# TzuYaoHuang/WaterLily.jl

Hardware: AMD Instinct MI355X
Metric: cells*steps/sec (3D TGV) ; smoother HBM GB/s vs peak (higher is better)
Workload: dtype f32; 1 GPU; 3D Taylor-Green vortex 512^3 Float32, wall-bounded, Re=1600, NoBody, remeasure=false (BASELINE configs[4] domain on 1 GPU); size=512, resjac=630, resjac_redo=0

## Files before the change

### include/wlhip.h

```cpp
#ifndef WLHIP_H
#define WLHIP_H
#include <stddef.h>
#include <stdint.h>

#ifdef __cplusplus
extern "C" {
#endif

#define WL_EINVAL (-1)
#define WL_ENOGPU (-2)
#define WL_ELEVELS (-3)
#define WL_ECOMM (-4)

typedef struct wl_grid {
  int32_t D;
  int32_t nx, ny, nz;
  int32_t k0, k1;
  int32_t gk;
  int32_t gnz;
} wl_grid;

enum { WL_QUICK = 0, WL_VANLEER = 1, WL_CDS = 2 };

int wl_init(int device);
// ... 75 lines not shown
float* wl_mg_level_field(const wl_mg* mg, int level, const char* name);
int wl_mg_vcycle(wl_mg* mg, int level, float omega, void* stream);
int wl_mg_smooth(wl_mg* mg, int level, int it, float omega, void* stream);
int wl_mg_level_is_const(const wl_mg* mg, int level);
int wl_mg_smoother_kind(const wl_mg* mg, int level);
int wl_mg_set_fused(wl_mg* mg, int on);
int wl_mg_solve(wl_mg* mg, double tol, int itmx, int* host_n, double* host_r1, float* host_rinf, void* stream);
int wl_mg_history(const wl_mg* mg, int16_t* host_out, int cap);
int wl_mg_last_log(const wl_mg* mg, double* host_r1, double* host_rinf, double* host_omega, int cap);
int wl_mg_shift_path(const wl_mg* mg);

typedef struct wl_sim wl_sim;
typedef struct wl_sim_desc {
  int32_t D;
  int32_t dims[3];
  float uBC[3];
  float nu, dt0;
  uint32_t perdir_mask;
  int32_t exitBC;
  int32_t scheme;
  int32_t has_body;
  float *u, *u0, *f, *p, *sigma, *V, *mu0, *mu1;
  float *us;
} wl_sim_desc;
int wl_sim_create(wl_sim** out, const wl_sim_desc* desc);
int wl_sim_create_on(wl_sim** out, const wl_sim_desc* desc, wl_mg* mg);
int wl_sim_destroy(wl_sim* s);
float* wl_sim_field(wl_sim* s, const char* name);
wl_mg* wl_sim_pois(wl_sim* s);
int wl_sim_grid(const wl_sim* s, wl_grid* out);
int wl_sim_init_flow(wl_sim* s, void* stream);
int wl_sim_set_option(wl_sim* s, const char* name, int value);
int wl_reset_process_options(void);
int wl_sim_set_forcing(wl_sim* s, const float* U1, const float* a0, const float* a1);
int wl_accelerate(float* r, const wl_grid* g, const float a[3], void* stream);
int wl_sim_set_sgs(wl_sim* s, int model, float Cs, float Delta);
int wl_sim_update(wl_sim* s, void* stream);
int wl_sim_mom_step(wl_sim* s, void* stream);
int wl_sim_mom_steps(wl_sim* s, int n, void* stream);
int wl_sim_dt(const wl_sim* s, float* host_out, int cap);
double wl_sim_time(const wl_sim* s);
float wl_sim_dt_last(const wl_sim* s);
int wl_sim_set_dt_last(wl_sim* s, float dt);
int wl_sim_phase(wl_sim* s, int phase, void* stream);
int wl_sim_apply_ic(wl_sim* s, int kind, void* stream);
int wl_sim_measure_sphere(wl_sim* s, const float* host_center, float R, float eps, void* stream);
enum { WL_BODY_SPHERE = 1, WL_BODY_PLANE = 2 };
typedef struct wl_body { int32_t kind; float c[3]; float R; float m[3]; float V[3]; } wl_body;
int wl_measure_body(float* sigma, float* mu0, float* mu1, float* V, const wl_grid* g, const wl_body* host_body, float eps, int exitBC, uint32_t perdir_mask, void* stream);
int wl_pressure_force_body(const float* p, const wl_grid* g, const wl_body* host_body, double out[3], void* stream);
int wl_viscous_force_body(const float* u, const wl_grid* g, float nu, const wl_body* host_body, double out[3], void* stream);
int wl_pressure_moment_body(const float* host_x0, const float* p, const wl_grid* g, const wl_body* host_body, double out[3], void* stream);
int wl_viscous_moment_body(const float* host_x0, const float* u, const wl_grid* g, float nu, const wl_body* host_body, double out[3], void* stream);
int wl_sim_pressure_moment_body(wl_sim* s, const float* host_x0, const wl_body* host_body, double out[3], void* stream);
int wl_sim_viscous_moment_body(wl_sim* s, const float* host_x0, const wl_body* host_body, double out[3], void* stream);
int wl_sim_measure_body(wl_sim* s, const wl_body* host_body, float eps, void* stream);
int wl_sim_pressure_force_body(wl_sim* s, const wl_body* host_body, double out[3], void* stream);
int wl_sim_viscous_force_body(wl_sim* s, const wl_body* host_body, double out[3], void* stream);
int wl_sim_pressure_force_sphere(wl_sim* s, const float* host_center, float R, double* host_out, void* stream);
int wl_sim_viscous_force_sphere(wl_sim* s, const float* center, float R, double* out, void* stream);

int wl_sim_flow_stats(wl_sim* s, const float* host_U, double out[3], void* stream);
int wl_sim_flow_fields(wl_sim* s, const float* host_U, float* ke, float* omega3, float* omega_mag, float* lambda2, void* stream);

int wl_interp(float* out, const float* arr, const wl_grid* g, const float* x, size_t n, int ncomp, void* hip_stream);
int wl_sim_sample(wl_sim* s, const float* x, size_t n, float* u_out, float* p_out, void* hip_stream);
// ... 66 lines not shown
```

### waterlily.jl_amd/__init__.py

```python
from ._lib import LIB_PATH, SIGNATURES, WlError, lib
from .core import (BC_, CDS, QUICK, VANLEER, L2, exitBC_, inside, jl_zeros, loc, perBC_, to_device, to_host)
from .flow import BDIM_, CFL, Flow, conv_diff_, mom_correct_, mom_predict_, mom_project_, mom_step_, scale_u_, sgs, sgs_, udf_
from .poisson import (pcg_, poisson_solver_, GaussSeidelRB_, Jacobi_, L1, Linf, MultiLevelPoisson, Poisson, increment_, mult_, norms, prolongate_,
                      residual_, restrict_, restrictL_, set_diag_, smooth_, update_)
from .metrics import (MeanFlow, curl_, flow_fields_, flow_stats, helicity_, ke_, lambda2_, load_checkpoint, omega_, omega_mag_, omega_theta_,
                      save_checkpoint)
from .interp import advect_, interp, interp_
from .simulation import (FusedSimulation, Simulation, measure_, pressure_force, pressure_moment, viscous_force,
                         viscous_moment)
from . import bodies
from .bodies import Body, RigidMap, SdfLattice, SetBody, setmap
```

### waterlily.jl_amd/_lib.py

```python
import ctypes as C
import os

_HERE = os.path.dirname(os.path.abspath(__file__))
LIB_PATH = os.environ.get("WLHIP_LIB") or os.path.join(_HERE, "libwlhip.so")


class wl_grid(C.Structure):
    _fields_ = [("D", C.c_int32), ("nx", C.c_int32), ("ny", C.c_int32), ("nz", C.c_int32),
                ("k0", C.c_int32), ("k1", C.c_int32), ("gk", C.c_int32), ("gnz", C.c_int32)]


class wl_body(C.Structure):
    _fields_ = [("kind", C.c_int32), ("c", C.c_float * 3), ("R", C.c_float), ("m", C.c_float * 3), ("V", C.c_float * 3)]


def make_body(body, D):
    name = body[0]
    pad = lambda v: [float(x) for x in v] + [0.0] * (3 - len(v))
    b = wl_body()
    if name == "sphere":
        b.kind, b.R, m, rest = 1, float(body[2]), [1.0] * D, body[3:]
    elif name == "cylinder":
        b.kind, b.R, m, rest = 1, float(body[2]), [0.0 if k == int(body[3]) else 1.0 for k in range(D)], body[4:]
    elif name == "plane":
# ... 118 lines not shown
    "wl_sim_set_forcing": (i32, [P, C.POINTER(f32), C.POINTER(f32), C.POINTER(f32)]),
    "wl_accelerate": (i32, [P, G, C.POINTER(f32), P]),
    "wl_sim_set_sgs": (i32, [P, i32, f32, f32]),
    "wl_sim_mom_step": (i32, [P, P]),
    "wl_sim_mom_steps": (i32, [P, i32, P]),
    "wl_sim_dt": (i32, [P, C.POINTER(f32), i32]),
    "wl_sim_time": (f64, [P]),
    "wl_sim_dt_last": (f32, [P]),
    "wl_sim_set_dt_last": (i32, [P, f32]),
    "wl_sim_phase": (i32, [P, i32, P]),
    "wl_sim_apply_ic": (i32, [P, i32, P]),
    "wl_sim_measure_sphere": (i32, [P, C.POINTER(f32), f32, f32, P]),
    "wl_comm_rccl_unique_id": (i32, [C.c_char_p]),
    "wl_comm_rccl_create": (i32, [C.POINTER(P), i32, i32, C.c_char_p]),
    "wl_comm_callbacks_create": (i32, [C.POINTER(P), i32, i32, P, P, P]),
    "wl_comm_rccl_available": (i32, []),
    "wl_comm_rccl_add_async": (i32, [P, C.c_char_p]),
    "wl_comm_set_loopback": (i32, [P, i32]),
    "wl_comm_set_virtual": (i32, [P, i32, i32]),
    "wl_comm_set_virtual_transport": (i32, [P, i32]),
    "wl_comm_set_periodic": (i32, [P, i32]),
    "wl_comm_halo_async": (i32, [P, P, G, i32, i32, P]),
    "wl_comm_combine_test": (i32, [P, P, P, P]),
    "wl_comm_destroy": (i32, [P]),
    "wl_comm_rank": (i32, [P]),
    "wl_comm_size": (i32, [P]),
    "wl_comm_stats": (i32, [P, C.POINTER(C.c_int64)]),
    "wl_halo_exchange": (i32, [P, P, G, i32, i32, P]),
    "wl_allgather_planes": (i32, [P, P, G, i32, P]),
    "wl_grid_slab": (i32, [G, i32, C.POINTER(C.c_int32), i32, i32, i32]),
    "wl_sim_create_slab": (i32, [C.POINTER(P), C.POINTER(wl_sim_desc), P]),
    "wl_launch_count": (C.c_long, []),
    "wl_reset_process_options": (i32, []),
    "wl_placement_scores": (i32, [C.POINTER(C.c_double), i32]),
    "wl_sim_counter": (i32, [P, C.c_char_p, C.POINTER(C.c_long)]),
    "wl_prof_enable": (i32, [i32]),
    "wl_prof_read": (i32, [i32, C.POINTER(i32), C.POINTER(f64)]),
    "wl_sim_pressure_force_sphere": (i32, [P, C.POINTER(f32), f32, C.POINTER(f64), P]),
    "wl_measure_body": (i32, [P, P, P, P, G, C.POINTER(wl_body), f32, i32, C.c_uint32, P]),
    "wl_pressure_force_body": (i32, [P, G, C.POINTER(wl_body), C.POINTER(f64), P]),
    "wl_viscous_force_body": (i32, [P, G, f32, C.POINTER(wl_body), C.POINTER(f64), P]),
    "wl_pressure_moment_body": (i32, [C.POINTER(f32), P, G, C.POINTER(wl_body), C.POINTER(f64), P]),
    "wl_viscous_moment_body": (i32, [C.POINTER(f32), P, G, f32, C.POINTER(wl_body), C.POINTER(f64), P]),
    "wl_sim_pressure_moment_body": (i32, [P, C.POINTER(f32), C.POINTER(wl_body), C.POINTER(f64), P]),
    "wl_sim_viscous_moment_body": (i32, [P, C.POINTER(f32), C.POINTER(wl_body), C.POINTER(f64), P]),
    "wl_sim_measure_body": (i32, [P, C.POINTER(wl_body), f32, P]),
    "wl_sim_pressure_force_body": (i32, [P, C.POINTER(wl_body), C.POINTER(f64), P]),
    "wl_sim_viscous_force_body": (i32, [P, C.POINTER(wl_body), C.POINTER(f64), P]),
    "wl_bodyset_measure_points": (i32, [C.POINTER(wl_bodyset), i32, C.POINTER(f32), i32, f32, C.POINTER(f32), C.POINTER(f32), C.POINTER(f32), P]),
    "wl_measure_bodyset": (i32, [P, P, P, P, G, C.POINTER(wl_bodyset), f32, i32, C.c_uint32, P]),
    "wl_pressure_force_bodyset": (i32, [C.POINTER(f32), P, G, C.POINTER(wl_bodyset), C.POINTER(f64), P]),
    "wl_viscous_force_bodyset": (i32, [C.POINTER(f32), P, G, f32, C.POINTER(wl_bodyset), C.POINTER(f64), P]),
    "wl_sim_measure_bodyset": (i32, [P, C.POINTER(wl_bodyset), f32, P]),
    "wl_sim_pressure_force_bodyset": (i32, [P, C.POINTER(f32), C.POINTER(wl_bodyset), C.POINTER(f64), P]),
    "wl_sim_viscous_force_bodyset": (i32, [P, C.POINTER(f32), C.POINTER(wl_bodyset), C.POINTER(f64), P]),
    "wl_sim_viscous_force_sphere": (i32, [P, C.POINTER(f32), f32, C.POINTER(f64), P]),
    "wl_sdf_lattice_create": (i32, [C.POINTER(P), i32, C.POINTER(C.c_int32), C.POINTER(f32), P]),
    "wl_sdf_lattice_destroy": (i32, [P]),
    "wl_sdf_lattice_id": (i32, [P]),
    "wl_sim_set_force_record": (i32, [P, C.POINTER(wl_bodyset), C.POINTER(f32), i32]),
    "wl_sim_read_forces": (i32, [P, C.POINTER(f64), i32, C.POINTER(i32), C.POINTER(i32)]),
    "wl_sim_forces_bodyset": (i32, [P, C.POINTER(f32), C.POINTER(wl_bodyset), C.POINTER(f64), P]),
    "wl_interp": (i32, [P, P, G, P, sz, i32, P]),
    "wl_sim_sample": (i32, [P, P, sz, P, P, P]),
    "wl_sim_set_probes": (i32, [P, C.POINTER(f32), i32, i32]),
    "wl_sim_read_probes": (i32, [P, C.POINTER(f32), i32, C.POINTER(i32), C.POINTER(i32)]),
# ... 36 lines not shown
```

### waterlily.jl_amd/csrc/wl_common.hpp

```cpp
#pragma once
#include <functional>
#include <cstdlib>
#include <hip/hip_runtime.h>
#include <stdint.h>

#include <mutex>
#include <string>
#include <vector>

#include "../../include/wlhip.h"
#include "../../include/wlhip_bench.h"

#define WL_WAVE 64
#define WL_BLOCK 256

void wl_set_error(const std::string& s);
#define WL_HIP(call)                                                                      \
  do {                                                                                    \
    hipError_t e__ = (call);                                                              \
    if (e__ != hipSuccess) {                                                              \
      wl_set_error(std::string(#call) + ": " + hipGetErrorString(e__));                   \
      return (int)e__;                                                                    \
    }                                                                                     \
  } while (0)
// ... 214 lines not shown
                   float dt, float pre, float post, const ConstL& cl, hipStream_t s, int ka = -(1 << 30), int kb = 1 << 30, bool q1 = true, BcFold* fold = nullptr);
int conv_q1(float* Phi, const float* u, const GridX& g, float nu, unsigned per, int scheme, hipStream_t s);
bool conv_z_ok(const GridX& g, unsigned per);
int conv_diff_z(float* f, const float* u_adv, const float* u0, const float* mu0, float* u_out, const GridX& g, float nu, int scheme, float dt, float pre, float post, hipStream_t s);
int bdim(float* u, const float* u0, float* f, const float* V, const float* mu0, const float* mu1, const GridX& g, float dt, float pre, float post, hipStream_t s);
int accelerate(float* r, const GridX& g, const float* a, hipStream_t s);
int exit_bc_single(const GridX& G, float* u, const float* u0, double* sc, float dt, hipStream_t s);
int exit_bc_slab_sum(const GridX& G, const float* u, double* sum, int mode, hipStream_t s);
int exit_bc_slab_update(const GridX& G, float* u, const float* u0, const double* gsum, double* sc, float dt, int mode, hipStream_t s);
int copy_exit_face(float* dst, const float* src, const GridX& G, hipStream_t s);
int sgs(float* f, float* sigma, const float* u, const GridX& g, float Cs, float Delta, hipStream_t s);
int metrics_fields(const float* u, const GridX& g, const float* U, float* ke, float* w3, float* wmag, float* l2, hipStream_t s);
int metrics_omega_theta(float* out, const float* u, const GridX& g, const float* z, const float* c, hipStream_t s);
int metrics_curl(float* out, const float* u, const GridX& g, int i, hipStream_t s);
int metrics_helicity(float* out, const float* u, const float* w3, const GridX& g, hipStream_t s);
int metrics_stats_dev(const float* u, const GridX& g, const float* U, const RedWs& ws, hipStream_t s);
int interp_points(const float* vec, const float* sca, const GridX& g, const float* x, size_t n, float* out_v, long ldv, float* out_s, long lds, hipStream_t s);
int advect(float* x, float* x_prev, const float* u0, const float* u1, const GridX& g, size_t n, float dt, unsigned per, hipStream_t s);
int bc_vec_fn(float* a, const float* Ub, const GridX& g, int saveexit, unsigned per, hipStream_t s);
int add_field(float* r, const float* gfield, size_t n, hipStream_t s);
int meanflow_update(float* P, float* U, float* UU, const float* p, const float* u, const GridX& g, float e, hipStream_t s);
int meanflow_uu(float* tau, const float* UU, const float* U, const GridX& g, hipStream_t s);
int bc_zplanes(float* u, const GridX& g, float U2, hipStream_t s);
void conv_tile_enable(int on, int chunk);
void conv_tile_min(long tile_planes);
bool conv_tile_ok(const GridX& g, unsigned per, int nplanes);
int conv_tile(const float* u_adv, const GridX& g, float nu, int scheme, int ka, int kb, const void* bdim_args, hipStream_t s);
void conv_flux_enable(int on);
bool conv_flux_on();
bool conv_proj_ok(const GridX& g, unsigned per);
int conv_flux(const float* u_adv, const GridX& g, float nu, int scheme, int ka, int kb, int zchunk, const void* bdim_args, hipStream_t s);
void conv_march_enable(int on);
void jacobi_march_enable(int on);
bool conv_march_ok(const GridX& g);
int conv_march(float* r, const float* u, const GridX& g, float nu, unsigned per, int scheme, int kfirst, int klast, const void* bdim_args, hipStream_t s);
int bdim_f(float* f, const float* u0, const float* V, const GridX& g, float dt, hipStream_t s);
int bdim_u(float* u, const float* f, const float* V, const float* mu0, const float* mu1, const GridX& g, float pre, float post, hipStream_t s, const unsigned char* far = nullptr);
size_t body_mask_bytes(const GridX& g);
int conv_diff_bdim_body(float* f, const float* u_adv, float* Phi, const float* u0, const float* mu0, float* u_out, const GridX& g, float nu, unsigned per, int scheme,
                        float dt, float pre, float post, const unsigned char* near, const unsigned char* needf, const unsigned char* m0var, int nbm, int store_all, hipStream_t s,
                        int dz0 = 0, int dz1 = -1);
struct MaskCensus { long near = 0, needf_only = 0, m0var_only = 0, clean_in_box = 0; };
int body_masks_planes(const unsigned char* near, const unsigned char* needf, const unsigned char* m0var, const GridX& g, int* dz, hipStream_t s,
                      const int* box = nullptr, MaskCensus* census = nullptr);
void conv_body_tile_enable(int on);
long conv_body_tile_launches();
int body_masks_nbm(const GridX& g);
int body_masks(unsigned char* near, unsigned char* needf, unsigned char* m0var, const float* V, const float* mu1, const float* mu0, const GridX& g, hipStream_t s);
int bdim_near(float* uout, const float* uin, const float* u0, float* f, const float* V, const float* mu0, const float* mu1, const GridX& g, float dt, float pre, float post,
              const unsigned char* near, int nbm, const int* box, hipStream_t s);
int body_masks_box(const unsigned char* near, const GridX& g, int* box, hipStream_t s);
int body_mask(unsigned char* far, const float* V, const float* mu1, const GridX& g, hipStream_t s);
int scale_u(float* u, const GridX& g, float sc, hipStream_t s);
int div(float* z, const float* u, const GridX& g, hipStream_t s);
int div_scale(float* z, float* x, const float* u, const GridX& g, float dt, hipStream_t s);
int project(float* u, const float* L, const float* x, const GridX& g, hipStream_t s);
int cfl_dev(const float* u, float* sigma, const GridX& g, const RedWs& ws, int slot_f, hipStream_t s);

int set_diag(float* D, float* iD, const float* L, const GridX& g, hipStream_t s);
int mult(float* z, const float* L, const float* D, const float* x, const GridX& g, hipStream_t s);
int residual(float* r, const float* x, const float* z, const float* L, const float* D, const float* iD, const GridX& g, const RedWs& ws, hipStream_t s);
int residual_part(float* r, const float* x, const float* z, const float* L, const float* D, const float* iD, const GridX& g, const RedWs& ws, hipStream_t s);
int mean_shift(float* r, const GridX& g, const RedWs& ws, hipStream_t s);
int div_residual(float* z, float* xout, float* r, const float* x, const float* u, const float* L, const float* D, const float* iD, const GridX& g, float dt, const RedWs& ws, const ConstL& cl, hipStream_t s);
int div_residual_split(float* z, float* xout, float* r, const float* x, const float* u, const float* L, const float* D, const float* iD, const GridX& g, float dt, const RedWs& ws,
                       const ConstL& near, const ConstL& far, int na, int nb, hipStream_t s);
// ... 56 lines not shown
```

### waterlily.jl_amd/csrc/wl_poisson.hip

```cpp
#include <vector>

#include "wl_common.hpp"
#include "wl_bcfold.hpp"
#include "wl_pdefer.hpp"

namespace {

template <int D>
__device__ __forceinline__ float Ax(const GridX& g, long o, const float* __restrict__ L, const float* __restrict__ Dg, const float* __restrict__ x) {
  float s = x[o] * Dg[o];
  s += (x[o - 1] * L[o] + x[o + 1] * L[o + 1]);
  s += (x[o - g.sy] * L[g.cs + o] + x[o + g.sy] * L[g.cs + o + g.sy]);
  if (D == 3) s += (x[o - g.sz] * L[2 * g.cs + o] + x[o + g.sz] * L[2 * g.cs + o + g.sz]);
  return s;
}

template <int D>
__global__ void k_set_diag(GridX g, float* __restrict__ Dg, float* __restrict__ iD, const float* __restrict__ L) {
  int i, j; long m; int pz;
  wl_tile(g, m, pz);
  if (!cell_ij(g, m, i, j) || !interior_ij(g, i, j)) return;
  const long o = m + (long)(g.k0 + pz) * g.sz;
  float s = 0.f;
  s -= (L[o] + L[o + 1]);
// ... 581 lines not shown
  float s = r[o];
  s -= (E(o - 1) * L[o] + E(o + 1) * L[o + 1]);
  s -= (E(o - g.sy) * L[g.cs + o] + E(o + g.sy) * L[g.cs + o + g.sy]);
  if (D == 3) s -= (E(o - g.sz) * L[2 * g.cs + o] + E(o + g.sz) * L[2 * g.cs + o + g.sz]);
  eps[o] = s * iD[o];
}
template <int D>
__global__ void k_jacobi_pp_cl(GridX g, float* __restrict__ rout, const float* __restrict__ r, float* __restrict__ x, float w, wl::ConstL cl, int xzero) {
  __shared__ float sDt[27], siDt[27];
  if (threadIdx.x < 27) { sDt[threadIdx.x] = cl.Dt[threadIdx.x]; siDt[threadIdx.x] = cl.iDt[threadIdx.x]; }
  __syncthreads();
  int i, j; long m; int pz;
  wl_tile(g, m, pz);
  if (!cell_ij(g, m, i, j) || !interior_ij(g, i, j)) return;
  const int k = g.k0 + pz;
  const long o = m + (long)k * g.sz;
  const int I0 = i + 1, I1 = j + 1, I2 = (D == 3) ? g.gk + k + 1 : 3;
  const int N2 = (D == 3) ? g.gnz : 8;
  const int cx0 = wl::wl_cl_cnt(I0, g.nx), cxm = wl::wl_cl_cnt(I0 - 1, g.nx), cxp = wl::wl_cl_cnt(I0 + 1, g.nx);
  const int cy0 = wl::wl_cl_cnt(I1, g.ny), cym = wl::wl_cl_cnt(I1 - 1, g.ny), cyp = wl::wl_cl_cnt(I1 + 1, g.ny);
  const int cz0 = (D == 3) ? wl::wl_cl_cnt(I2, N2) : 0, czm = (D == 3) ? wl::wl_cl_cnt(I2 - 1, N2) : 0, czp = (D == 3) ? wl::wl_cl_cnt(I2 + 1, N2) : 0;
  const float lx = wl::wl_cl_coef(I0, g.nx, cl.c[0]), lxp = wl::wl_cl_coef(I0 + 1, g.nx, cl.c[0]);
  const float ly = wl::wl_cl_coef(I1, g.ny, cl.c[1]), lyp = wl::wl_cl_coef(I1 + 1, g.ny, cl.c[1]);
  const float lz = (D == 3) ? wl::wl_cl_coef(I2, N2, cl.c[2]) : 0.f, lzp = (D == 3) ? wl::wl_cl_coef(I2 + 1, N2, cl.c[2]) : 0.f;
  auto ID = [&](int a, int b, int c) -> float { return siDt[a + 3 * b + 9 * c]; };
  const float e0 = r[o] * ID(cx0, cy0, cz0);
  float s = e0 * sDt[cx0 + 3 * cy0 + 9 * cz0];
  s += ((r[o - 1] * ID(cxm, cy0, cz0)) * lx + (r[o + 1] * ID(cxp, cy0, cz0)) * lxp);
  s += ((r[o - g.sy] * ID(cx0, cym, cz0)) * ly + (r[o + g.sy] * ID(cx0, cyp, cz0)) * lyp);
  if (D == 3) s += ((r[o - g.sz] * ID(cx0, cy0, czm)) * lz + (r[o + g.sz] * ID(cx0, cy0, czp)) * lzp);
  rout[o] = r[o] - w * s;
  x[o] = (xzero ? 0.f : x[o]) + w * e0;
}
template <int SHIFT>
__global__ void k_jacobi_march_cl(GridX g, float* __restrict__ rout, const float* __restrict__ r, float* __restrict__ x, float w, wl::ConstL cl, int zchunk,
                                  const double* __restrict__ sum, double n_inside, double* __restrict__ part, float* __restrict__ pmax, int xzero) {
  __shared__ float sDt[27], siDt[27];
  if (threadIdx.x < 27) { sDt[threadIdx.x] = cl.Dt[threadIdx.x]; siDt[threadIdx.x] = cl.iDt[threadIdx.x]; }
  __syncthreads();
  int i, j; long m; int pz;
  wl_tile(g, m, pz);
  float c = 0.f;
  if (SHIFT) c = wl_shift_due(*sum, n_inside) ? wl_shift_mean(*sum, n_inside) : 0.f;
  float acc = 0.f, mx = 0.f;
  const int ks = g.k0 + pz * zchunk, ke = (ks + zchunk < g.k1) ? ks + zchunk : g.k1;
  const bool live = cell_ij(g, m, i, j) && interior_ij(g, i, j) && ks < ke;
  if (!SHIFT && !live) return;
  if (live) {
  const int I0 = i + 1, I1 = j + 1;
  const int cx0 = wl::wl_cl_cnt(I0, g.nx), cxm = wl::wl_cl_cnt(I0 - 1, g.nx), cxp = wl::wl_cl_cnt(I0 + 1, g.nx);
  const int cy0 = wl::wl_cl_cnt(I1, g.ny), cym = wl::wl_cl_cnt(I1 - 1, g.ny), cyp = wl::wl_cl_cnt(I1 + 1, g.ny);
  const float lx = wl::wl_cl_coef(I0, g.nx, cl.c[0]), lxp = wl::wl_cl_coef(I0 + 1, g.nx, cl.c[0]);
  const float ly = wl::wl_cl_coef(I1, g.ny, cl.c[1]), lyp = wl::wl_cl_coef(I1 + 1, g.ny, cl.c[1]);
  float d0[3], id0[3], idxm[3], idxp[3], idym[3], idyp[3];
#pragma unroll
  for (int c = 0; c < 3; c++) {
    d0[c] = sDt[cx0 + 3 * cy0 + 9 * c]; id0[c] = siDt[cx0 + 3 * cy0 + 9 * c];
    idxm[c] = siDt[cxm + 3 * cy0 + 9 * c]; idxp[c] = siDt[cxp + 3 * cy0 + 9 * c];
    idym[c] = siDt[cx0 + 3 * cym + 9 * c]; idyp[c] = siDt[cx0 + 3 * cyp + 9 * c];
  }
  auto pick = [](const float* t, int c) -> float { return c == 2 ? t[2] : (c == 1 ? t[1] : t[0]); };
  long o = m + (long)ks * g.sz;
  float rm = r[o - g.sz] - c, r0 = r[o] - c;
  for (int k = ks; k < ke; k++, o += g.sz) {
    const float rp = r[o + g.sz] - c;
    if (SHIFT) { const float av = fabsf(r0); acc += av; mx = fmaxf(mx, av); }
    const int I2 = g.gk + k + 1;
    const int cz0 = wl::wl_cl_cnt(I2, g.gnz), czm = wl::wl_cl_cnt(I2 - 1, g.gnz), czp = wl::wl_cl_cnt(I2 + 1, g.gnz);
    const float lz = wl::wl_cl_coef(I2, g.gnz, cl.c[2]), lzp = wl::wl_cl_coef(I2 + 1, g.gnz, cl.c[2]);
    const float e0 = r0 * pick(id0, cz0);
    float s = e0 * pick(d0, cz0);
    s += (((r[o - 1] - c) * pick(idxm, cz0)) * lx + ((r[o + 1] - c) * pick(idxp, cz0)) * lxp);
    s += (((r[o - g.sy] - c) * pick(idym, cz0)) * ly + ((r[o + g.sy] - c) * pick(idyp, cz0)) * lyp);
    s += ((rm * pick(id0, czm)) * lz + (rp * pick(id0, czp)) * lzp);
    rout[o] = r0 - w * s;
    x[o] = (xzero ? 0.f : x[o]) + w * e0;
    rm = r0; r0 = rp;
  }
  }
  if (SHIFT) {
    const double accd = block_sum((double)acc); mx = block_max(mx);
    if (threadIdx.x == 0) { part[blockIdx.x] = accd; pmax[blockIdx.x] = mx; }
  }
}
template <int D>
__global__ void k_jacobi_pp(GridX g, float* __restrict__ rout, const float* __restrict__ r, float* __restrict__ x, const float* __restrict__ L,
                            const float* __restrict__ Dg, const float* __restrict__ iD, float w, int xzero) {
  int i, j; long m; int pz;
  wl_tile(g, m, pz);
  if (!cell_ij(g, m, i, j) || !interior_ij(g, i, j)) return;
  const int k = g.k0 + pz;
  const long o = m + (long)k * g.sz;
  auto E = [&](long oo) -> float { return r[oo] * iD[oo]; };
  const float e0 = r[o] * iD[o];
  const float lx = L[o], lxp = L[o + 1], ly = L[g.cs + o], lyp = L[g.cs + o + g.sy];
  const float lz = (D == 3) ? L[2 * g.cs + o] : 0.f, lzp = (D == 3) ? L[2 * g.cs + o + g.sz] : 0.f;
  float dgv = 0.f;
  dgv -= (lx + lxp);
  dgv -= (ly + lyp);
  if (D == 3) dgv -= (lz + lzp);
  float s = e0 * dgv;
  s += (E(o - 1) * lx + E(o + 1) * lxp);
  s += (E(o - g.sy) * ly + E(o + g.sy) * lyp);
  if (D == 3) s += (E(o - g.sz) * lz + E(o + g.sz) * lzp);
  rout[o] = r[o] - w * s;
  x[o] = (xzero ? 0.f : x[o]) + w * e0;
}
__global__ void k_shift_norms(GridX g, float* __restrict__ r, const double* __restrict__ sum, double n_inside, double* __restrict__ part, float* __restrict__ pmax) {
  int i, j; long m; int pz;
  wl_tile(g, m, pz);
  const float s = wl_shift_mean(*sum, n_inside);
  const bool shift = wl_shift_due(*sum, n_inside);
  double acc = 0.0; float mx = 0.f;
  const int nsl = wl_nslots(g);
  if (cell_ij(g, m, i, j) && interior_ij(g, i, j)) {
    for (int k = g.k0 + pz; k < g.k1; k += nsl) {
      const long o = m + (long)k * g.sz;
// ... 588 lines not shown
  hipLaunchKernelGGL(k_final_sum_max, dim3(1), dim3(WL_BLOCK), 0, s, ws.pa, ws.pm, nparts, ws.res_d + slot_d, ws.res_f + slot_f);
  WL_LAUNCH_CHECK(); return 0;
}
int increment(float* r, float* x, const float* eps, const float* L, const float* Dg, const GridX& g, float w, hipStream_t s) {
  DSEL(g.D, k_increment, wl_plane_grid(g, g.k1 - g.k0), dim3(WL_BLOCK), 0, s, g, r, x, eps, L, Dg, w);
  WL_LAUNCH_CHECK(); return 0;
}
int jacobi(float* eps, float* r, float* x, const float* L, const float* Dg, const float* iD, const GridX& g, float w, bool write_eps, hipStream_t s) {
  (void)write_eps;
  hipLaunchKernelGGL(k_gs_init, wl_plane_grid(g, g.k1 - g.k0), dim3(WL_BLOCK), 0, s, g, eps, r, iD);
  WL_LAUNCH_CHECK();
  return increment(r, x, eps, L, Dg, g, w, s);
}
int gs_init(float* eps, const float* r, const float* iD, const GridX& g, hipStream_t s) {
  hipLaunchKernelGGL(k_gs_init, wl_plane_grid(g, g.k1 - g.k0), dim3(WL_BLOCK), 0, s, g, eps, r, iD);
  WL_LAUNCH_CHECK(); return 0;
}
int gs_init_sweep1(float* eps, const float* r, const float* L, const float* iD, const GridX& g, hipStream_t s) {
  DSEL(g.D, k_gs_init_sweep1, wl_plane_grid(g, g.k1 - g.k0), dim3(WL_BLOCK), 0, s, g, eps, r, L, iD);
  WL_LAUNCH_CHECK(); return 0;
}
static int g_jacobi_march = 1;
void jacobi_march_enable(int on) { g_jacobi_march = on; }
bool jacobi_takes_shift(const GridX& g, const ConstL& cl) { return cl.on && g.D == 3 && g_jacobi_march && g.nz == g.gnz; }
int jacobi_pp_shift(float* rout, const float* r, float* x, const GridX& g, float w, const ConstL& cl, const RedWs& ws, int slot_d, int slot_f, hipStream_t s) {
  if (!jacobi_takes_shift(g, cl)) { wl_set_error("jacobi_pp_shift: level not eligible"); return WL_EINVAL; }
  const int zc = wl_march_chunk(g, g.k1 - g.k0);
  dim3 grid = wl_plane_grid(g, wl_march_slots(g.k1 - g.k0, zc));
  const double ni = (double)wl_ninside_global(wl_grid{g.D, g.nx, g.ny, g.nz, g.k0, g.k1, g.gk, g.gnz});
  hipLaunchKernelGGL(k_jacobi_march_cl<1>, grid, dim3(WL_BLOCK), 0, s, g, rout, r, x, w, cl, zc, (const double*)(ws.res_d + WL_RD_SUM), ni, ws.pa, ws.pm, 0);
  hipLaunchKernelGGL(k_final_sum_max, dim3(1), dim3(WL_BLOCK), 0, s, ws.pa, ws.pm, (int)grid.x, ws.res_d + slot_d, ws.res_f + slot_f);
  WL_LAUNCH_CHECK(); return 0;
}
int jacobi_pp(float* rout, const float* r, float* x, const float* L, const float* Dg, const float* iD, const GridX& g, float w, const ConstL& cl, hipStream_t s, int xzero) {
  if (cl.on && g.D == 3 && g_jacobi_march) {
    const int zc = wl_march_chunk(g, g.k1 - g.k0);
    hipLaunchKernelGGL(k_jacobi_march_cl<0>, wl_plane_grid(g, wl_march_slots(g.k1 - g.k0, zc)), dim3(WL_BLOCK), 0, s, g, rout, r, x, w, cl, zc, (const double*)nullptr, 0.0, (double*)nullptr, (float*)nullptr, xzero);
  } else if (cl.on) DSEL(g.D, k_jacobi_pp_cl, wl_plane_grid(g, g.k1 - g.k0), dim3(WL_BLOCK), 0, s, g, rout, r, x, w, cl, xzero);
  else DSEL(g.D, k_jacobi_pp, wl_plane_grid(g, g.k1 - g.k0), dim3(WL_BLOCK), 0, s, g, rout, r, x, L, Dg, iD, w, xzero);
  WL_LAUNCH_CHECK(); return 0;
}
int g_tail_lds = 1;
void tail_lds_enable(int on) { g_tail_lds = on; }
int vcycle_tail(const TailLevelHost* lv, int n, float w, hipStream_t s) {
  if (n < 1 || n > WL_TAIL_MAXLV) { wl_set_error("vcycle_tail: bad level count"); return WL_EINVAL; }
  TailArgsL b; TailArgs& a = b.a; a.n = n; a.w = w;
  for (int l = 0; l < n; l++) a.lv[l] = TailLevel{lv[l].g, lv[l].L, lv[l].D, lv[l].iD, lv[l].x, lv[l].eps, lv[l].r, lv[l].cx, lv[l].cy, lv[l].cz};
  bool cl = true, fits = g_tail_lds != 0;
  long lo = 54 * WL_TAIL_MAXLV;
  for (int l = 0; l < n; l++) {
    const GridX& g = lv[l].g;
    if (g.D != 3 || g.gk != 0 || g.nz != g.gnz || g.nx < 3 || g.ny < 3 || g.nz < 3 || g.cs > WL_TAIL_CELLS) fits = false;
    if ((long)(g.nx - 2) * (g.ny - 2) * (g.nz - 2) > 4096) fits = false;
    cl = cl && lv[l].cl && lv[l].cl->on;
    b.q[l].lo = (int)lo; b.q[l].inx = 1.f / (float)(g.nx - 2); b.q[l].iny = 1.f / (float)(g.ny - 2);
    for (int c = 0; c < 3; c++) b.q[l].c[c] = (lv[l].cl && lv[l].cl->on) ? lv[l].cl->c[c] : 0.f;
    for (int t = 0; t < 27; t++) { b.tab[54 * l + t] = (lv[l].cl && lv[l].cl->on) ? lv[l].cl->Dt[t] : 0.f; b.tab[54 * l + 27 + t] = (lv[l].cl && lv[l].cl->on) ? lv[l].cl->iDt[t] : 0.f; }
    lo += 3 * g.cs;
  }
  const size_t bytes = (size_t)lo * sizeof(float);
  if (fits && bytes <= 156 * 1024) {
    static bool attr[2] = {false, false};
    if (!attr[cl ? 1 : 0]) {
      WL_HIP(cl ? hipFuncSetAttribute((const void*)k_vcycle_tail_lds<true>, hipFuncAttributeMaxDynamicSharedMemorySize, 156 * 1024)
                : hipFuncSetAttribute((const void*)k_vcycle_tail_lds<false>, hipFuncAttributeMaxDynamicSharedMemorySize, 156 * 1024));
      attr[cl ? 1 : 0] = true;
    }
    if (cl) hipLaunchKernelGGL(k_vcycle_tail_lds<true>, dim3(1), dim3(1024), bytes, s, b);
// ... 50 lines not shown
```

### waterlily.jl_amd/csrc/wl_sim.hip

```cpp
#include <cmath>
#include <cstring>
#include <utility>
#include <vector>

#include "wl_common.hpp"
#include <algorithm>
#include "wl_mg.hpp"
#include "wl_body.hpp"
#include "wl_pdefer.hpp"
#include "wl_forces.hpp"
#include "wl_meanflow.hpp"
#include "wl_observe.hpp"

namespace {
template <int D>
__global__ void k_apply_tgv(GridX g, float* __restrict__ u, float kx, float ky, float kz) {
  int i, j; long m; int pz;
  wl_tile(g, m, pz);
  if (!cell_ij(g, m, i, j)) return;
  const int k = pz;
  const long o = m + (long)k * g.sz;
  const int I[3] = {i + 1, j + 1, (D == 3) ? g.gk + k + 1 : 1};
  for (int a = 0; a < D; a++) {
    float x[3];
// ... 608 lines not shown
  if (n == "overlap") { WL_TRY(s->sync_u(0)); s->use_overlap = value != 0; return 0; }
  if (n == "fuse_cfl") { s->use_fuse_cfl = value != 0; return 0; }
  if (n == "jacobi_march") { wl::jacobi_march_enable(value); return 0; }
  if (n == "convm") { wl::conv_march_enable(value); return 0; }
  if (n == "deep_halo") { s->mg->deep_halo = value != 0; return 0; }
  if (n == "x_halo") { if (value < 1 || value > s->G.k0) { wl_set_error("x_halo: 1 .. ghost depth of the slab"); return WL_EINVAL; } s->mg->x_halo_depth = value; return 0; }
  if (n == "bcfold") { s->use_bcfold = value; return 0; }
  if (n == "resjac") { s->use_resjac = value != 0; s->resjac_force_redo = value == 2 || value == 3; s->redo_unannounced = value == 3; return 0; }
  if (n == "resjac_min") { wl::resjac_enable(1, value); return 0; }
  if (n == "convt_min") { wl::conv_tile_min(value); return 0; }
  if (n == "lazydt") { s->use_lazydt = value != 0; return 0; }
  if (n == "tailspec") { s->use_tailspec = value != 0; return 0; }
  if (n == "headspec") { s->use_headspec = value != 0; return 0; }
  if (n == "bcdefer") { s->use_bcdefer = value != 0; return 0; }
  if (n == "pdefer") { s->use_pdefer = value != 0; return 0; }
  if (n == "rskip") { WL_TRY(s->mg->settle_r_for_reader()); s->mg->skip_r = value != 0; return 0; }
  if (n == "tailwide") { s->use_tailwide = value != 0; return 0; }
  if (n == "tailfuse") { s->use_tailfuse = value != 0; if (value != 0) s->tailfuse_min = 0; return 0; }
  if (n == "tailfuse_min") { if (value < 0) { wl_set_error("tailfuse_min: interior cells, >= 0"); return WL_EINVAL; } s->tailfuse_min = value; return 0; }
  if (n == "convf") { wl::conv_flux_enable(value != 0); return 0; }
  if (n == "convt") { wl::conv_tile_enable(value != 0, value > 1 ? value : 0); return 0; }
  if (n == "pair") { wl::gsrb_pair_enable(value); return 0; }
  if (n == "fuse_p") { s->use_fuse_p = value != 0; return 0; }
  if (n == "zsplit_par") { s->mg->par_ranges = value != 0; return 0; }
  if (n == "itmx") { if (value < 1) { wl_set_error("itmx must be >= 1"); return WL_EINVAL; } s->itmx = value; return 0; }
  wl_set_error("unknown option " + n); return WL_EINVAL;
}
int wl_sim_update(wl_sim* s, void* st) { s->resjac_backoff = false; s->resjac_redo_run = 0; WL_TRY(s->refresh_body_mask(wl_stream(st))); return s->mg->update(wl_stream(st)); }

long wl_launch_count(void) { return g_wl_launches; }
int wl_reset_process_options(void) {
  wl::resjac_enable(1, 6L << 20); wl::conv_tile_min(2048); wl::conv_tile_enable(1, 0); wl::conv_flux_enable(1); wl::tail_lds_enable(1); wl::conv_body_tile_enable(1);
  wl::gsrb_pair_enable(1); wl::jacobi_march_enable(1); wl::conv_march_enable(0);
  return 0;
}
int wl_sim_counter(wl_sim* s, const char* name, long* out) {
  WL_CHECK(s && name && out, "bad argument");
  const std::string n(name);
  if (n == "resjac") { *out = s->n_resjac; return 0; }
  if (n == "resjac_redo") { *out = s->n_resjac_redo; return 0; }
  if (n == "resjac_backoff") { *out = s->resjac_backoff ? 1 : 0; return 0; }
  if (n == "tailfuse") { *out = s->n_tailfuse; return 0; }
  if (n == "tailfuse_min") { *out = s->tailfuse_min; return 0; }
  if (n == "bcdefer") { *out = s->n_bcdefer; return 0; }
  if (n == "pdefer") { *out = s->n_pdefer; return 0; }
  if (n == "tailwide") { *out = s->n_tailwide; return 0; }
  if (n == "rskip") { *out = s->mg->n_rskip; return 0; }
  if (n == "rskip_redo") { *out = s->mg->n_rskip_redo; return 0; }
  if (n == "tailspec") { *out = s->n_tailspec; return 0; }
  if (n == "tailspec_armed") { *out = s->n_tailspec_armed; return 0; }
  if (n == "xdefer") { *out = s->mg->last_xdefer; return 0; }
  if (n == "abwide") { *out = s->mg->n_wide; return 0; }
  if (n == "hybrid") { *out = s->n_hybrid; return 0; }
  if (n == "body_tile") { *out = wl::conv_body_tile_launches(); return 0; }
  if (n == "mask_valid") { *out = s->mask_valid ? 1 : 0; return 0; }
  if (n == "mask_near") { *out = s->census.near; return 0; }
  if (n == "mask_needf_only") { *out = s->census.needf_only; return 0; }
  if (n == "mask_m0var_only") { *out = s->census.m0var_only; return 0; }
  if (n == "mask_clean_in_box") { *out = s->census.clean_in_box; return 0; }
  if (n == "dirty_z0") { *out = s->dirty_z[0]; return 0; }
  if (n == "dirty_z1") { *out = s->dirty_z[1]; return 0; }
  if (n == "near_b0") { *out = s->near_box[0]; return 0; }
  if (n == "near_b1") { *out = s->near_box[1]; return 0; }
  if (n == "near_k0") { *out = s->near_box[2]; return 0; }
  if (n == "near_k1") { *out = s->near_box[3]; return 0; }
  if (n == "part") { *out = s->mg->lv[0].part ? 1 : 0; return 0; }
  if (n == "part_za") { *out = s->mg->lv[0].za; return 0; }
// ... 226 lines not shown
```

### waterlily.jl_amd/poisson.py

```python
import ctypes as C

import numpy as np

from . import core
from ._lib import WlError, check, lib, wl_grid
from .core import jl_zeros, perBC_, perdir_mask, ptr, sgrid, stream


class Poisson:

    def __init__(self, x, L, z, perdir=()):
        assert tuple(x.shape) == tuple(z.shape) and tuple(L.shape) == tuple(x.shape) + (x.dim(),)
        self.x, self.L, self.z = x, L, z
        self.perdir = tuple(perdir)
        self.r, self.eps, self.D, self.iD = (jl_zeros(tuple(x.shape)) for _ in range(4))
        self.n = []
        self.g = sgrid(x)
        set_diag_(self.D, self.iD, self.L)

    def n_inside(self):
        return int(np.prod([s - 2 for s in self.x.shape]))


def set_diag_(D, iD, L):
# ... 26 lines not shown


def GaussSeidelRB_(p, it=4, w=1.0):
    check(lib().wl_gsrb(ptr(p.eps), ptr(p.r), ptr(p.x), ptr(p.L), ptr(p.D), ptr(p.iD), C.byref(p.g), int(it), float(w), perdir_mask(p.perdir), stream()))


smooth_ = GaussSeidelRB_


def pcg_(p, it=6):
    check(lib().wl_pcg(ptr(p.eps), ptr(p.r), ptr(p.x), ptr(p.z), ptr(p.L), ptr(p.D), ptr(p.iD), C.byref(p.g), int(it), perdir_mask(p.perdir), stream()))


def poisson_solver_(p, tol=2e-3, itmx=1e3):
    n, r1, rinf = C.c_int(), C.c_double(), C.c_float()
    check(lib().wl_poisson_solve(ptr(p.eps), ptr(p.r), ptr(p.x), ptr(p.z), ptr(p.L), ptr(p.D), ptr(p.iD), C.byref(p.g), float(tol), int(itmx),
                                 perdir_mask(p.perdir), C.byref(n), C.byref(r1), C.byref(rinf), stream()))
    p.n.append(n.value)
    return n.value


def norms(p):
    l1, linf = C.c_double(), C.c_float()
    check(lib().wl_norms(ptr(p.r), C.byref(p.g), C.byref(l1), C.byref(linf), None, stream()))
    return np.float32(l1.value), np.float32(linf.value)


def L1(p):
    return norms(p)[0]


def Linf(p):
    return norms(p)[1]


def restrict_(a, b):
    ga, gb = sgrid(a), sgrid(b)
    check(lib().wl_restrict(ptr(a), C.byref(ga), ptr(b), C.byref(gb), stream()))


def prolongate_(a, b):
    ga, gb = sgrid(a), sgrid(b)
    check(lib().wl_prolongate(ptr(a), C.byref(ga), ptr(b), C.byref(gb), stream()))


def restrictL_(a, b, perdir=()):
    ga, gb = core.vgrid(a), core.vgrid(b)
    check(lib().wl_restrictL(ptr(a), C.byref(ga), ptr(b), C.byref(gb), perdir_mask(perdir), stream()))


class _LevelView:

    def __init__(self, ml, l):
        self._ml, self._l = ml, l
        g = wl_grid()
        check(lib().wl_mg_level_grid(ml._h, l, C.byref(g)))
        self.grid = g
        self.dims = (g.nx, g.ny) if g.D == 2 else (g.nx, g.ny, g.nz)

    def _get(self, name):
        D = len(self.dims)
        shape = self.dims + (D,) if name == "L" else self.dims
        out = np.empty(shape, dtype=np.float32, order="F")
        p = lib().wl_mg_level_field(self._ml._h, self._l, name.encode())
        check(lib().wl_d2h(out.ctypes.data_as(C.c_void_p), p, out.nbytes, stream()))
        return out
# ... 85 lines not shown
```

Before: 17.62 billion cells*steps/s.

## Add LDS-tiled z-marching Jacobi smoother kernel for constant-coefficient 3D levels

```diff
diff --git a/include/wlhip.h b/include/wlhip.h
--- a/include/wlhip.h
+++ b/include/wlhip.h
@@ -131,6 +131,8 @@
 int wl_sim_init_flow(wl_sim* s, void* stream);
 int wl_sim_set_option(wl_sim* s, const char* name, int value);
 int wl_reset_process_options(void);
+int wl_set_process_option(const char* name, int value);
+int wl_process_counter(const char* name, long* out);
 int wl_sim_set_forcing(wl_sim* s, const float* U1, const float* a0, const float* a1);
 int wl_accelerate(float* r, const wl_grid* g, const float a[3], void* stream);
 int wl_sim_set_sgs(wl_sim* s, int model, float Cs, float Delta);
diff --git a/waterlily.jl_amd/__init__.py b/waterlily.jl_amd/__init__.py
--- a/waterlily.jl_amd/__init__.py
+++ b/waterlily.jl_amd/__init__.py
@@ -1,8 +1,8 @@
 from ._lib import LIB_PATH, SIGNATURES, WlError, lib
 from .core import (BC_, CDS, QUICK, VANLEER, L2, exitBC_, inside, jl_zeros, loc, perBC_, to_device, to_host)
 from .flow import BDIM_, CFL, Flow, conv_diff_, mom_correct_, mom_predict_, mom_project_, mom_step_, scale_u_, sgs, sgs_, udf_
-from .poisson import (pcg_, poisson_solver_, GaussSeidelRB_, Jacobi_, L1, Linf, MultiLevelPoisson, Poisson, increment_, mult_, norms, prolongate_,
-                      residual_, restrict_, restrictL_, set_diag_, smooth_, update_)
+from .poisson import (pcg_, poisson_solver_, process_counter, GaussSeidelRB_, Jacobi_, L1, Linf, MultiLevelPoisson, Poisson, increment_, mult_, norms, prolongate_,
+                      residual_, restrict_, restrictL_, set_diag_, set_process_option, smooth_, update_)
 from .metrics import (MeanFlow, curl_, flow_fields_, flow_stats, helicity_, ke_, lambda2_, load_checkpoint, omega_, omega_mag_, omega_theta_,
                       save_checkpoint)
 from .interp import advect_, interp, interp_
diff --git a/waterlily.jl_amd/_lib.py b/waterlily.jl_amd/_lib.py
--- a/waterlily.jl_amd/_lib.py
+++ b/waterlily.jl_amd/_lib.py
@@ -174,6 +174,8 @@
     "wl_sim_create_slab": (i32, [C.POINTER(P), C.POINTER(wl_sim_desc), P]),
     "wl_launch_count": (C.c_long, []),
     "wl_reset_process_options": (i32, []),
+    "wl_set_process_option": (i32, [C.c_char_p, i32]),
+    "wl_process_counter": (i32, [C.c_char_p, C.POINTER(C.c_long)]),
     "wl_placement_scores": (i32, [C.POINTER(C.c_double), i32]),
     "wl_sim_counter": (i32, [P, C.c_char_p, C.POINTER(C.c_long)]),
     "wl_prof_enable": (i32, [i32]),
diff --git a/waterlily.jl_amd/csrc/wl_common.hpp b/waterlily.jl_amd/csrc/wl_common.hpp
--- a/waterlily.jl_amd/csrc/wl_common.hpp
+++ b/waterlily.jl_amd/csrc/wl_common.hpp
@@ -270,6 +270,8 @@
 int conv_flux(const float* u_adv, const GridX& g, float nu, int scheme, int ka, int kb, int zchunk, const void* bdim_args, hipStream_t s);
 void conv_march_enable(int on);
 void jacobi_march_enable(int on);
+void jacobi_tile_enable(int on);
+long jacobi_tile_launches();
 bool conv_march_ok(const GridX& g);
 int conv_march(float* r, const float* u, const GridX& g, float nu, unsigned per, int scheme, int kfirst, int klast, const void* bdim_args, hipStream_t s);
 int bdim_f(float* f, const float* u0, const float* V, const GridX& g, float dt, hipStream_t s);
diff --git a/waterlily.jl_amd/csrc/wl_poisson.hip b/waterlily.jl_amd/csrc/wl_poisson.hip
--- a/waterlily.jl_amd/csrc/wl_poisson.hip
+++ b/waterlily.jl_amd/csrc/wl_poisson.hip
@@ -637,6 +637,15 @@
   rout[o] = r[o] - w * s;
   x[o] = (xzero ? 0.f : x[o]) + w * e0;
 }
+__device__ __forceinline__ float jacobi_cell(float r0, float rxm, float rxp, float rym, float ryp, float rzm, float rzp, float id0, float d0, float idxm, float idxp,
+                                             float idym, float idyp, float idzm, float idzp, float lx, float lxp, float ly, float lyp, float lz, float lzp, float w, float& e0) {
+  e0 = r0 * id0;
+  float s = e0 * d0;
+  s += ((rxm * idxm) * lx + (rxp * idxp) * lxp);
+  s += ((rym * idym) * ly + (ryp * idyp) * lyp);
+  s += ((rzm * idzm) * lz + (rzp * idzp) * lzp);
+  return r0 - w * s;
+}
 template <int SHIFT>
 __global__ void k_jacobi_march_cl(GridX g, float* __restrict__ rout, const float* __restrict__ r, float* __restrict__ x, float w, wl::ConstL cl, int zchunk,
                                   const double* __restrict__ sum, double n_inside, double* __restrict__ part, float* __restrict__ pmax, int xzero) {
@@ -673,12 +682,9 @@
     const int I2 = g.gk + k + 1;
     const int cz0 = wl::wl_cl_cnt(I2, g.gnz), czm = wl::wl_cl_cnt(I2 - 1, g.gnz), czp = wl::wl_cl_cnt(I2 + 1, g.gnz);
     const float lz = wl::wl_cl_coef(I2, g.gnz, cl.c[2]), lzp = wl::wl_cl_coef(I2 + 1, g.gnz, cl.c[2]);
-    const float e0 = r0 * pick(id0, cz0);
-    float s = e0 * pick(d0, cz0);
-    s += (((r[o - 1] - c) * pick(idxm, cz0)) * lx + ((r[o + 1] - c) * pick(idxp, cz0)) * lxp);
-    s += (((r[o - g.sy] - c) * pick(idym, cz0)) * ly + ((r[o + g.sy] - c) * pick(idyp, cz0)) * lyp);
-    s += ((rm * pick(id0, czm)) * lz + (rp * pick(id0, czp)) * lzp);
-    rout[o] = r0 - w * s;
+    float e0;
+    rout[o] = jacobi_cell(r0, r[o - 1] - c, r[o + 1] - c, r[o - g.sy] - c, r[o + g.sy] - c, rm, rp, pick(id0, cz0), pick(d0, cz0), pick(idxm, cz0), pick(idxp, cz0),
+                          pick(idym, cz0), pick(idyp, cz0), pick(id0, czm), pick(id0, czp), lx, lxp, ly, lyp, lz, lzp, w, e0);
     x[o] = (xzero ? 0.f : x[o]) + w * e0;
     rm = r0; r0 = rp;
   }
@@ -688,6 +694,109 @@
     if (threadIdx.x == 0) { part[blockIdx.x] = accd; pmax[blockIdx.x] = mx; }
   }
 }
+#define WL_JT_X 64
+#define WL_JT_Y 16
+#define WL_JT_LD 68
+#define WL_JT_THREADS (WL_JT_X / 2 * WL_JT_Y)
+struct jt_pair { float x, y; };
+__device__ __forceinline__ float2 jt_ld2(const float* p) { const jt_pair v = *reinterpret_cast<const jt_pair*>(p); return make_float2(v.x, v.y); }
+__device__ __forceinline__ void jt_st2(float* p, float2 v) { *reinterpret_cast<jt_pair*>(p) = jt_pair{v.x, v.y}; }
+static inline int jacobi_tile_count(const GridX& g) { return ((g.nx - 2 + WL_JT_X - 1) / WL_JT_X) * ((g.ny - 2 + WL_JT_Y - 1) / WL_JT_Y); }
+__global__ void __launch_bounds__(WL_JT_THREADS) k_jacobi_tile(GridX g, float* __restrict__ rout, const float* __restrict__ r, float* __restrict__ x, float w, wl::ConstL cl,
+                                                                int zchunk, int xzero) {
+  __shared__ float sDt[27], siDt[27];
+  __shared__ __attribute__((aligned(16))) float sh[2][WL_JT_Y + 2][WL_JT_LD];
+  const int t = threadIdx.x;
+  if (t < 27) { sDt[t] = cl.Dt[t]; siDt[t] = cl.iDt[t]; }
+  const int ntx = (g.nx - 2 + WL_JT_X - 1) / WL_JT_X, ntile = ntx * ((g.ny - 2 + WL_JT_Y - 1) / WL_JT_Y);
+  const unsigned per = (unsigned)((ntile + 7) >> 3), hs = blockIdx.x >> 3;
+  const int pz = (int)(hs / per), tile = (int)((blockIdx.x & 7u) * per + (hs - (unsigned)pz * per));
+  const int ks = g.k0 + pz * zchunk, ke = (ks + zchunk < g.k1) ? ks + zchunk : g.k1;
+  if (tile >= ntile || ks >= ke) return;
+  const int i0 = 1 + (tile % ntx) * WL_JT_X, j0 = 1 + (tile / ntx) * WL_JT_Y;
+  const int tx = t & 31, ty = t >> 5;
+  const int ia = i0 + 2 * tx, j = j0 + ty;
+  const bool va = ia <= g.nx - 2 && j <= g.ny - 2, vb = va && ia + 1 <= g.nx - 2;
+  struct Src { long o; bool sh; };
+  auto src = [&](int i, int jj) -> Src {
+    const int ic = i < g.nx - 2 ? i : g.nx - 2, jc = jj < g.ny - 1 ? jj : g.ny - 1;
+    return Src{(long)ic + (long)jc * g.sy, i == g.nx - 1};
+  };
+  const Src sc = src(ia, j);
+  const bool ringw = __builtin_amdgcn_readfirstlane(t >> 6) < 2;
+  int gmode = 0, gl = 0; Src sg = sc;
+  if (t < 64) {
+    const int gj = (t < 32) ? j0 - 1 : j0 + WL_JT_Y;
+    gmode = (gj <= g.ny - 1 && ia <= g.nx - 1) ? 2 : 0;
+    sg = src(ia, gj); gl = ((t < 32) ? 0 : WL_JT_Y + 1) * WL_JT_LD + 2 + 2 * tx;
+  } else if (t < 96) {
+    const int side = (t - 64) >> 4, gj = j0 + ((t - 64) & 15), gi = side ? i0 + WL_JT_X : i0 - 1;
+    gmode = (gj <= g.ny - 1 && gi <= g.nx - 1) ? 1 : 0;
+    sg = src(gi, gj); gl = (1 + ((t - 64) & 15)) * WL_JT_LD + (side ? WL_JT_X + 2 : 1);
+  }
+  auto load = [&](const float* __restrict__ a, const Src& q, int k) -> float2 {
+    return jt_ld2(a + q.o + (long)k * g.sz);
+  };
+  auto fix = [](float2 v, bool sh) -> float2 { if (sh) v.x = v.y; return v; };
+  const int cl_ = (ty + 1) * WL_JT_LD + 2 + 2 * tx;
+  auto stage = [&](int b, float2 c, float2 gv) {
+    float* p = &sh[b][0][0];
+    *reinterpret_cast<float2*>(p + cl_) = c;
+    if (gmode == 2) *reinterpret_cast<float2*>(p + gl) = gv; else if (gmode == 1) p[gl] = gv.x;
+  };
+  __syncthreads();
+  const int I0 = ia + 1, I1 = j + 1;
+  const int cy0 = wl::wl_cl_cnt(I1, g.ny), cym = wl::wl_cl_cnt(I1 - 1, g.ny), cyp = wl::wl_cl_cnt(I1 + 1, g.ny);
+  int cx[4];
+#pragma unroll
+  for (int q = 0; q < 4; q++) cx[q] = wl::wl_cl_cnt(I0 - 1 + q, g.nx);
+  const float lxa = wl::wl_cl_coef(I0, g.nx, cl.c[0]), lxb = wl::wl_cl_coef(I0 + 1, g.nx, cl.c[0]), lxc = wl::wl_cl_coef(I0 + 2, g.nx, cl.c[0]);
+  const float ly = wl::wl_cl_coef(I1, g.ny, cl.c[1]), lyp = wl::wl_cl_coef(I1 + 1, g.ny, cl.c[1]);
+  float idx[4][3], d0[2][3], idym[2][3], idyp[2][3];
+#pragma unroll
+  for (int c = 0; c < 3; c++) {
+#pragma unroll
+    for (int q = 0; q < 4; q++) idx[q][c] = siDt[cx[q] + 3 * cy0 + 9 * c];
+#pragma unroll
+    for (int e = 0; e < 2; e++) { d0[e][c] = sDt[cx[1 + e] + 3 * cy0 + 9 * c]; idym[e][c] = siDt[cx[1 + e] + 3 * cym + 9 * c]; idyp[e][c] = siDt[cx[1 + e] + 3 * cyp + 9 * c]; }
+  }
+  auto pick3 = [](float t0, float t1, float t2, int c) -> float { return c == 2 ? t2 : (c == 1 ? t1 : t0); };
+#define JT_PICK(tb, c) pick3((tb)[0], (tb)[1], (tb)[2], c)
+  float2 zero2 = make_float2(0.f, 0.f);
+  float2 rm = fix(load(r, sc, ks - 1), sc.sh), r0 = fix(load(r, sc, ks), sc.sh);
+  stage(0, r0, fix(ringw ? load(r, sg, ks) : zero2, sg.sh));
+  float2 rpl = load(r, sc, ks + 1), gpl = ringw ? load(r, sg, ks + 1) : zero2;
+  float2 xpl = xzero ? zero2 : load(x, sc, ks);
+  __syncthreads();
+  long o = (long)ia + (long)j * g.sy + (long)ks * g.sz;
+  for (int k = ks; k < ke; k++, o += g.sz) {
+    const int b = (k - ks) & 1;
+    const float* p = &sh[b][0][0] + cl_;
+    const float rxm = p[-1], rxp = p[2];
+    const float2 rym = *reinterpret_cast<const float2*>(p - WL_JT_LD), ryp = *reinterpret_cast<const float2*>(p + WL_JT_LD);
+    const float2 rp = fix(rpl, sc.sh), xo = xpl;
+    stage(b ^ 1, rp, fix(gpl, sg.sh));
+    const int k2 = k + 2 <= ke ? k + 2 : ke, k1 = k + 1 < ke ? k + 1 : k;
+    rpl = load(r, sc, k2);
+    if (ringw) gpl = load(r, sg, k2);
+    if (!xzero) xpl = load(x, sc, k1);
+    if (va) {
+      const int I2 = g.gk + k + 1;
+      const int cz0 = wl::wl_cl_cnt(I2, g.gnz), czm = wl::wl_cl_cnt(I2 - 1, g.gnz), czp = wl::wl_cl_cnt(I2 + 1, g.gnz);
+      const float lz = wl::wl_cl_coef(I2, g.gnz, cl.c[2]), lzp = wl::wl_cl_coef(I2 + 1, g.gnz, cl.c[2]);
+      float2 ro, e;
+      ro.x = jacobi_cell(r0.x, rxm, r0.y, rym.x, ryp.x, rm.x, rp.x, JT_PICK(idx[1], cz0), JT_PICK(d0[0], cz0), JT_PICK(idx[0], cz0), JT_PICK(idx[2], cz0),
+                         JT_PICK(idym[0], cz0), JT_PICK(idyp[0], cz0), JT_PICK(idx[1], czm), JT_PICK(idx[1], czp), lxa, lxb, ly, lyp, lz, lzp, w, e.x);
+      ro.y = jacobi_cell(r0.y, r0.x, rxp, rym.y, ryp.y, rm.y, rp.y, JT_PICK(idx[2], cz0), JT_PICK(d0[1], cz0), JT_PICK(idx[1], cz0), JT_PICK(idx[3], cz0),
+                         JT_PICK(idym[1], cz0), JT_PICK(idyp[1], cz0), JT_PICK(idx[2], czm), JT_PICK(idx[2], czp), lxb, lxc, ly, lyp, lz, lzp, w, e.y);
+      const float2 xn = make_float2((xzero ? 0.f : xo.x) + w * e.x, (xzero ? 0.f : xo.y) + w * e.y);
+      if (vb) { jt_st2(rout + o, ro); jt_st2(x + o, xn); } else { rout[o] = ro.x; x[o] = xn.x; }
+    }
+    rm = r0; r0 = rp;
+    __syncthreads();
+  }
+}
+#undef JT_PICK
 template <int D>
 __global__ void k_jacobi_pp(GridX g, float* __restrict__ rout, const float* __restrict__ r, float* __restrict__ x, const float* __restrict__ L,
                             const float* __restrict__ Dg, const float* __restrict__ iD, float w, int xzero) {
@@ -1342,8 +1451,26 @@
   hipLaunchKernelGGL(k_final_sum_max, dim3(1), dim3(WL_BLOCK), 0, s, ws.pa, ws.pm, (int)grid.x, ws.res_d + slot_d, ws.res_f + slot_f);
   WL_LAUNCH_CHECK(); return 0;
 }
+static long g_n_jacobi_tile = 0;
+static int g_jacobi_tile = 1;
+void jacobi_tile_enable(int on) { g_jacobi_tile = on; }
+long jacobi_tile_launches() { return g_n_jacobi_tile; }
+static int jacobi_tile_chunk(const GridX& g) {
+  if (!g_jacobi_tile || g.gk != 0 || g.nz != g.gnz || g.k0 != 1 || g.k1 != g.nz - 1) return 0;
+  const long np = g.k1 - g.k0, bp = 8L * ((jacobi_tile_count(g) + 7) >> 3);
+  static const long groups = [] { const long v = wl_exp_int("WL_JT_GROUPS", 2048); return v >= 1 ? v : 2048; }();
+  static const long gate = wl_exp_int("WL_JT_MIN_GROUPS", 512);
+  long c = np * bp / groups; if (c > 32) c = 32; if (c < 4) c = 4; if (c > np) c = np;
+  if ((np + c - 1) / c * bp < gate && g_jacobi_tile != 2) return 0;
+  return (int)c;
+}
 int jacobi_pp(float* rout, const float* r, float* x, const float* L, const float* Dg, const float* iD, const GridX& g, float w, const ConstL& cl, hipStream_t s, int xzero) {
-  if (cl.on && g.D == 3 && g_jacobi_march) {
+  const int tc = (cl.on && g.D == 3 && g_jacobi_march) ? jacobi_tile_chunk(g) : 0;
+  if (tc) {
+    const unsigned nb = 8u * (unsigned)((jacobi_tile_count(g) + 7) >> 3) * (unsigned)wl_march_slots(g.k1 - g.k0, tc);
+    g_n_jacobi_tile++;
+    hipLaunchKernelGGL(k_jacobi_tile, dim3(nb), dim3(WL_JT_THREADS), 0, s, g, rout, r, x, w, cl, tc, xzero);
+  } else if (cl.on && g.D == 3 && g_jacobi_march) {
     const int zc = wl_march_chunk(g, g.k1 - g.k0);
     hipLaunchKernelGGL(k_jacobi_march_cl<0>, wl_plane_grid(g, wl_march_slots(g.k1 - g.k0, zc)), dim3(WL_BLOCK), 0, s, g, rout, r, x, w, cl, zc, (const double*)nullptr, 0.0, (double*)nullptr, (float*)nullptr, xzero);
   } else if (cl.on) DSEL(g.D, k_jacobi_pp_cl, wl_plane_grid(g, g.k1 - g.k0), dim3(WL_BLOCK), 0, s, g, rout, r, x, w, cl, xzero);
diff --git a/waterlily.jl_amd/csrc/wl_sim.hip b/waterlily.jl_amd/csrc/wl_sim.hip
--- a/waterlily.jl_amd/csrc/wl_sim.hip
+++ b/waterlily.jl_amd/csrc/wl_sim.hip
@@ -664,7 +664,23 @@
 int wl_reset_process_options(void) {
   wl::resjac_enable(1, 6L << 20); wl::conv_tile_min(2048); wl::conv_tile_enable(1, 0); wl::conv_flux_enable(1); wl::tail_lds_enable(1); wl::conv_body_tile_enable(1);
   wl::gsrb_pair_enable(1); wl::jacobi_march_enable(1); wl::conv_march_enable(0);
+  wl::jacobi_tile_enable(1);
   return 0;
+}
+int wl_set_process_option(const char* name, int value) {
+  WL_CHECK(name, "bad argument");
+  const std::string n(name);
+  if (n == "jacobi_tile") {
+    if (value < 0 || value > 2) { wl_set_error("jacobi_tile: 0, 1 or 2"); return WL_EINVAL; }
+    wl::jacobi_tile_enable(value); return 0;
+  }
+  wl_set_error("unknown process option " + n); return WL_EINVAL;
+}
+int wl_process_counter(const char* name, long* out) {
+  WL_CHECK(name && out, "bad argument");
+  const std::string n(name);
+  if (n == "jacobi_tile") { *out = wl::jacobi_tile_launches(); return 0; }
+  wl_set_error("unknown process counter " + n); return WL_EINVAL;
 }
 int wl_sim_counter(wl_sim* s, const char* name, long* out) {
   WL_CHECK(s && name && out, "bad argument");
diff --git a/waterlily.jl_amd/poisson.py b/waterlily.jl_amd/poisson.py
--- a/waterlily.jl_amd/poisson.py
+++ b/waterlily.jl_amd/poisson.py
@@ -82,6 +82,16 @@
 
 def Linf(p):
     return norms(p)[1]
+
+
+def set_process_option(name, value):
+    check(lib().wl_set_process_option(str(name).encode(), int(value)))
+
+
+def process_counter(name):
+    v = C.c_long()
+    check(lib().wl_process_counter(str(name).encode(), C.byref(v)))
+    return int(v.value)
 
 
 def restrict_(a, b):
```

Measured after the change: 17.59 billion cells*steps/s. Within noise of the previous version (-0.2%).
